# stanford-iprl-lab/nerf_shared

Hardware: AMD Instinct MI355X
Metric: rays_per_sec (higher is better)
Workload: dtype bf16; 1 GPU; lego_halfres_400x400_64c+128f_viewdirs_8x256_chunk4096; entry=Renderer.render(c2w=pose, retraw=False), chunk=4096, N_samples=64, N_importance=128, weights=random-init seeds 0/10, parallelism=single GPU

## Files before the change

include/nerf_amd.h:

```cpp
#ifndef NERF_AMD_H
#define NERF_AMD_H

#include <stdint.h>

#ifdef __cplusplus
extern "C" {
#endif

#define NERF_AMD_ABI_VERSION 7

#define NERF_AMD_OK            0
#define NERF_AMD_EINVAL       -1
#define NERF_AMD_EHIP         -2
#define NERF_AMD_EUNSUPPORTED -3
#define NERF_AMD_ENOMEM       -4

#define NERF_AMD_PREC_FP32 0
#define NERF_AMD_PREC_BF16 1
#define NERF_AMD_PREC_FP32_SPLIT 2

#define NERF_AMD_SPLIT_TRAIN_MAX_POINTS 8388352

#define NERF_AMD_MAX_SKIPS 8

// ... 210 lines not shown
                              void *stream);

int nerf_amd_occupancy_cull(const nerf_amd_occupancy_grid *grid, const float *rays, int32_t ray_ch, const float *z, int64_t R,
                            int32_t S, int32_t *block_counts, int32_t *rank, float *pts_live, float *vd_live, int64_t *count,
                            void *stream);

int nerf_amd_occupancy_expand(const float *raw_live, const int32_t *rank, int64_t n, int32_t ch, float *raw, void *stream);

int nerf_amd_field_points(const nerf_amd_model *m, const float *pts, const float *viewdirs, int64_t n, float *raw,
                          int precision, void *stream);

int64_t nerf_amd_render_rays_culled_workspace(const nerf_amd_render_cfg *cfg, int64_t R, int32_t out_ch);
int     nerf_amd_render_rays_culled(const nerf_amd_render_cfg *cfg, const nerf_amd_model *coarse, const nerf_amd_model *fine,
                                    const nerf_amd_render_io *io, int64_t R, const nerf_amd_occupancy_grid *grid,
                                    int64_t *stats, void *stream);

int nerf_amd_to8b(const float *x, int64_t n, uint8_t *out, void *stream);

int nerf_amd_img2mse(const float *x, const float *y, int64_t n, float *out, float *partials, void *stream);
int nerf_amd_img2mse_backward(const float *x, const float *y, int64_t n, const float *g, float *gx, float *gy, void *stream);

int nerf_amd_assemble_rays(const float *rays_o, const float *rays_d, const float *viewdir_src, int64_t n, float near,
                           float far, float *out, void *stream);

int nerf_amd_adam_step(int32_t n, float *const *params, const float *const *grads, float *const *exp_avg,
                       float *const *exp_avg_sq, const int64_t *numel, int64_t step, double lr, double beta1,
                       double beta2, double eps, double weight_decay, void *stream);

int nerf_amd_adam_step_device(int32_t n, float *const *params, const float *const *grads, float *const *exp_avg,
                              float *const *exp_avg_sq, const int64_t *numel, int64_t *step_dev, const double *lr_dev,
                              double beta1, double beta2, double eps, double weight_decay, float *scalars_dev, void *stream);

int nerf_amd_profile_enable(int on);
int nerf_amd_set_tuning(int key, int value);
int nerf_amd_profile_collect(int64_t launches[3], double total_ms[3], double total_points[3]);

#ifdef __cplusplus
}
#endif
#endif
```

nerf_shared_amd/_lib.py:

```python
import ctypes
import os
from ctypes import POINTER, Structure, c_char_p, c_double, c_float, c_int, c_int32, c_int64, c_uint16, c_uint32, c_void_p

_HERE = os.path.dirname(os.path.abspath(__file__))
LIB_PATH = os.environ.get("NERF_AMD_LIB") or os.path.join(_HERE, "libnerf_amd.so")

ABI_VERSION = 7
PREC_FP32, PREC_BF16, PREC_FP32_SPLIT = 0, 1, 2
COPY_BF16, COPY_BWD, COPY_SPLIT, COPY_BWD_SPLIT, COPY_FP32, COPY_FP32_BWD, COPY_ALL = 1, 2, 4, 8, 16, 32, 63
COPY_BF16_FOLD = 128
COPY_OF = {PREC_BF16: COPY_BF16, PREC_FP32_SPLIT: COPY_SPLIT, PREC_FP32: COPY_FP32}
TRAIN_COPIES = {PREC_BF16: COPY_BF16 | COPY_BWD, PREC_FP32_SPLIT: COPY_SPLIT | COPY_BWD_SPLIT,
                PREC_FP32: COPY_FP32 | COPY_FP32_BWD}
MAX_SKIPS = 8

EXPORTS = (
    "nerf_amd_abi_version", "nerf_amd_last_error",
    "nerf_amd_model_create", "nerf_amd_model_update", "nerf_amd_model_update_copies", "nerf_amd_model_destroy",
    "nerf_amd_model_supports_bf16", "nerf_amd_model_supports_split", "nerf_amd_model_out_ch", "nerf_amd_pack_bf16_host",
    "nerf_amd_embed", "nerf_amd_nerf_forward", "nerf_amd_mlp_embedded", "nerf_amd_ndc_rays", "nerf_amd_raw2outputs", "nerf_amd_raw2outputs_backward", "nerf_amd_sample_pdf",
    "nerf_amd_render_rays_workspace", "nerf_amd_render_rays", "nerf_amd_render_chunks", "nerf_amd_make_rays",
    "nerf_amd_render_batch_workspace", "nerf_amd_render_batch",
    "nerf_amd_profile_enable", "nerf_amd_profile_collect", "nerf_amd_set_tuning",
    "nerf_amd_model_supports_training", "nerf_amd_train_workspace", "nerf_amd_field_forward_train",
    "nerf_amd_field_backward", "nerf_amd_coarse_z", "nerf_amd_resample", "nerf_amd_get_rays_backward", "nerf_amd_to8b", "nerf_amd_ndc_rays_backward", "nerf_amd_adam_step", "nerf_amd_adam_step_device", "nerf_amd_img2mse", "nerf_amd_img2mse_backward", "nerf_amd_assemble_rays",
    "nerf_amd_rays_at_pixels", "nerf_amd_rays_at_pixels_backward", "nerf_amd_se3_transform", "nerf_amd_se3_transform_backward",
    "nerf_amd_field_backward_inputs",
    "nerf_amd_se3_transform_batch", "nerf_amd_se3_transform_batch_backward", "nerf_amd_rays_at_pixels_batch",
    "nerf_amd_rays_at_pixels_batch_backward", "nerf_amd_img2mse_each", "nerf_amd_img2mse_each_backward",
    "nerf_amd_density_arch", "nerf_amd_density", "nerf_amd_density_grad_fused", "nerf_amd_density_grad_workspace",
    "nerf_amd_density_value_grad",
    "nerf_amd_draw_pixels", "nerf_amd_interest_points_workspace", "nerf_amd_interest_points", "nerf_amd_dilate_mask",
    "nerf_amd_compact_mask",
    "nerf_amd_occupancy_query", "nerf_amd_occupancy_sample_points", "nerf_amd_occupancy_mark", "nerf_amd_occupancy_dilate",
    "nerf_amd_occupancy_cull", "nerf_amd_occupancy_expand", "nerf_amd_field_points",
    "nerf_amd_render_rays_culled_workspace", "nerf_amd_render_rays_culled",
)
OCC_OUTSIDE_LIVE, OCC_OUTSIDE_EMPTY = 0, 1


class Arch(Structure):
    _fields_ = [("D", c_int32), ("W", c_int32), ("output_ch", c_int32), ("use_viewdirs", c_int32),
                ("multires", c_int32), ("multires_views", c_int32), ("i_embed", c_int32),
                ("n_skips", c_int32), ("skips", c_int32 * MAX_SKIPS)]


class RenderCfg(Structure):
    _fields_ = [("N_samples", c_int32), ("N_importance", c_int32), ("perturb", c_int32), ("lindisp", c_int32),
                ("white_bkgd", c_int32), ("use_noise", c_int32), ("precision", c_int32), ("reserved", c_int32)]


class RenderIO(Structure):
    _fields_ = [("rays", c_void_p), ("ray_ch", c_int32), ("pad0", c_int32),
                ("t_vals", c_void_p), ("t_rand", c_void_p), ("noise0", c_void_p), ("noise1", c_void_p),
                ("u", c_void_p), ("t_lin_imp", c_void_p), ("z_coarse", c_void_p),
                ("rgb_map", c_void_p), ("disp_map", c_void_p), ("acc_map", c_void_p),
# ... 80 lines not shown
        "nerf_amd_img2mse_each": (c_int, [c_void_p, c_void_p, c_int64, c_int64, c_int32, c_void_p, c_void_p]),
        "nerf_amd_img2mse_each_backward": (c_int, [c_void_p, c_void_p, c_int64, c_int64, c_int32, c_void_p, c_void_p, c_void_p]),
        "nerf_amd_draw_pixels": (c_int, [c_int64, c_int32, c_uint32, c_void_p, c_void_p, c_int32, c_int32, c_void_p, c_int64, c_int32,
                                         c_void_p, c_void_p, c_void_p]),
        "nerf_amd_interest_points_workspace": (c_int64, [c_int32, c_int32]),
        "nerf_amd_interest_points": (c_int, [c_void_p, c_int32, c_int32, c_int32, c_int32, c_void_p, c_void_p, c_void_p]),
        "nerf_amd_dilate_mask": (c_int, [c_void_p, c_int32, c_int32, c_int32, c_int32, c_void_p, c_void_p]),
        "nerf_amd_compact_mask": (c_int, [c_void_p, c_int32, c_int32, c_void_p, c_void_p, c_void_p, c_void_p]),
        "nerf_amd_occupancy_query": (c_int, [POINTER(OccupancyGridC), c_void_p, c_int64, c_void_p, c_void_p, c_void_p]),
        "nerf_amd_occupancy_sample_points": (c_int, [POINTER(OccupancyGridC), c_int64, c_int64, c_int32, c_uint32, c_void_p, c_void_p]),
        "nerf_amd_occupancy_mark": (c_int, [c_void_p, c_int64, c_int64, c_int32, c_float, c_int, c_void_p, c_void_p]),
        "nerf_amd_occupancy_dilate": (c_int, [c_void_p, c_int32, c_int32, c_int32, c_int32, c_void_p, c_void_p]),
        "nerf_amd_occupancy_cull": (c_int, [POINTER(OccupancyGridC), c_void_p, c_int32, c_void_p, c_int64, c_int32, c_void_p, c_void_p,
                                            c_void_p, c_void_p, c_void_p, c_void_p]),
        "nerf_amd_occupancy_expand": (c_int, [c_void_p, c_void_p, c_int64, c_int32, c_void_p, c_void_p]),
        "nerf_amd_field_points": (c_int, [c_void_p, c_void_p, c_void_p, c_int64, c_void_p, c_int, c_void_p]),
        "nerf_amd_render_rays_culled_workspace": (c_int64, [POINTER(RenderCfg), c_int64, c_int32]),
        "nerf_amd_render_rays_culled": (c_int, [POINTER(RenderCfg), c_void_p, c_void_p, POINTER(RenderIO), c_int64,
                                                POINTER(OccupancyGridC), POINTER(c_int64), c_void_p]),
        "nerf_amd_get_rays_backward": (c_int, [c_int32, c_int32, POINTER(c_double), c_int64, c_int64, c_void_p, c_void_p,
                                               c_void_p, c_void_p]),
        "nerf_amd_to8b": (c_int, [c_void_p, c_int64, c_void_p, c_void_p]),
        "nerf_amd_img2mse": (c_int, [c_void_p, c_void_p, c_int64, c_void_p, c_void_p, c_void_p]),
        "nerf_amd_img2mse_backward": (c_int, [c_void_p, c_void_p, c_int64, c_void_p, c_void_p, c_void_p, c_void_p]),
        "nerf_amd_assemble_rays": (c_int, [c_void_p, c_void_p, c_void_p, c_int64, c_float, c_float, c_void_p, c_void_p]),
        "nerf_amd_adam_step": (c_int, [c_int32, c_void_p, c_void_p, c_void_p, c_void_p, c_void_p, c_int64, c_double, c_double,
                               c_double, c_double, c_double, c_void_p]),
        "nerf_amd_adam_step_device": (c_int, [c_int32, c_void_p, c_void_p, c_void_p, c_void_p, c_void_p, c_void_p, c_void_p, c_double,
                                      c_double, c_double, c_double, c_void_p, c_void_p]),
        "nerf_amd_ndc_rays_backward": (c_int, [c_int32, c_int32, c_double, c_float, c_void_p, c_void_p, c_void_p, c_void_p,
                                               c_int64, c_void_p, c_void_p, c_void_p]),
        "nerf_amd_profile_enable": (c_int, [c_int]),
        "nerf_amd_profile_collect": (c_int, [POINTER(c_int64), POINTER(c_double), POINTER(c_double)]),
    }
    for name, (res, args) in sig.items():
        fn = getattr(lib, name)
        fn.restype, fn.argtypes = res, args
    if lib.nerf_amd_abi_version() != ABI_VERSION:
        raise ImportError("libnerf_amd.so ABI version %d, binding expects %d" % (lib.nerf_amd_abi_version(), ABI_VERSION))
    return lib


lib = _load()


class NerfAmdError(RuntimeError):
    pass


def check(rc, what):
    if rc != 0:
        msg = lib.nerf_amd_last_error()
        raise NerfAmdError("%s failed (%d): %s" % (what, rc, msg.decode() if msg else "?"))


def make_arch(D, W, output_ch, skips, use_viewdirs, multires, multires_views, i_embed):
    skips = [int(s) for s in skips]
    if len(skips) > MAX_SKIPS:
        raise ValueError("at most %d skip connections are supported" % MAX_SKIPS)
    a = Arch()
    a.D, a.W, a.output_ch, a.use_viewdirs = int(D), int(W), int(output_ch), int(bool(use_viewdirs))
    a.multires, a.multires_views, a.i_embed, a.n_skips = int(multires), int(multires_views), int(i_embed), len(skips)
    for i, s in enumerate(skips):
        a.skips[i] = s
    return a

# ... 15 lines not shown
```

nerf_shared_amd/csrc/capi.hip:

```cpp
#include <hip/hip_runtime.h>

#include <atomic>
#include <cmath>

#include <cstdio>
#include <cstring>
#include <mutex>
#include <utility>
#include <new>
#include <string>
#include <vector>

#include "kernels.h"
#include "launch_util.h"
#include "program.h"

using namespace na;

namespace {
thread_local std::string g_err;

std::string lds_msg(const char *what, size_t bytes) {
    return std::string(what) + ": the per-ray scratch needs " + std::to_string(bytes) + " bytes of LDS per workgroup, the CU has " +
           std::to_string(LDS_LIMIT_BYTES) + " (fewer samples per ray)";
}

int fail(int code, const std::string &msg) {
    g_err = msg;
    return code;
}
int hip_fail(hipError_t e, const char *what) {
    return fail(NERF_AMD_EHIP, std::string(what) + ": " + hipGetErrorString(e));
}
#define HIP_TRY(expr)                                        \
    do {                                                     \
        hipError_t e_ = (expr);                              \
        if (e_ != hipSuccess) return hip_fail(e_, #expr);    \
    } while (0)

struct ProfRec { hipEvent_t a, b; int cls; double points; };
std::mutex g_prof_mu;
bool g_prof_on = false;
std::vector<ProfRec> g_prof_recs;
std::vector<std::pair<hipEvent_t, hipEvent_t>> g_prof_free;

template <class T>
int upload(T **dst, const std::vector<T> &src) {
    *dst = nullptr;
    if (src.empty()) return NERF_AMD_OK;
    HIP_TRY(hipMalloc(reinterpret_cast<void **>(dst), src.size() * sizeof(T)));
    HIP_TRY(hipMemcpy(*dst, src.data(), src.size() * sizeof(T), hipMemcpyHostToDevice));
    return NERF_AMD_OK;
}
size_t align_up(size_t v) { return (v + 255) & ~(size_t)255; }

constexpr int TILE_CTR_SLOTS = 1024;
unsigned *g_tile_ctr[16] = {};
std::atomic<unsigned> g_tile_ctr_next{0};
}

namespace na {
std::atomic<int> g_variant{0};
std::atomic<int> g_fold{0};

int tile_counters_init(int device) {
    if (device < 0 || device >= 16) return NERF_AMD_EINVAL;
    if (g_tile_ctr[device]) return NERF_AMD_OK;
    unsigned *p = nullptr;
    if (hipMalloc(reinterpret_cast<void **>(&p), TILE_CTR_SLOTS * 2 * sizeof(unsigned)) != hipSuccess) return NERF_AMD_EHIP;
    if (hipMemset(p, 0, TILE_CTR_SLOTS * 2 * sizeof(unsigned)) != hipSuccess) { (void)hipFree(p); return NERF_AMD_EHIP; }
    g_tile_ctr[device] = p;
    return NERF_AMD_OK;
}

unsigned *tile_counter_slot(int device) {
    if (device < 0 || device >= 16 || !g_tile_ctr[device]) return nullptr;
    return g_tile_ctr[device] + 2 * (g_tile_ctr_next.fetch_add(1, std::memory_order_relaxed) % TILE_CTR_SLOTS);
}

unsigned *tile_counter_for(bool deal, hipStream_t s) {
    if (!deal) return nullptr;
    hipStreamCaptureStatus st = hipStreamCaptureStatusNone;
    if (hipStreamIsCapturing(s, &st) != hipSuccess || st != hipStreamCaptureStatusNone) return nullptr;
    int dev = 0;
    return hipGetDevice(&dev) == hipSuccess ? tile_counter_slot(dev) : nullptr;
}
}

struct nerf_amd_model {
    Program prog;
    int device = 0;
    FragDesc *d_frags = nullptr;
    TileDesc *d_tiles = nullptr;
    LayerF32 *d_layers = nullptr;
    TensorDesc *d_tensors = nullptr;
    uint16_t *stream_bf16 = nullptr, *stream_s16 = nullptr, *stream_bwd = nullptr, *stream_split = nullptr;
// ... 1026 lines not shown
    DeviceGuard guard(device);
    if (guard.err != hipSuccess) return hip_fail(guard.err, "hipSetDevice(lane device)");
    SideLane &l = g_lanes[device];
    if (!l.stream) HIP_TRY(hipStreamCreateWithFlags(&l.stream, hipStreamNonBlocking));
    out[0] = l.stream;
    for (int i = 1; i < n; ++i) {
        if (!l.more[i - 1]) HIP_TRY(hipStreamCreateWithFlags(&l.more[i - 1], hipStreamNonBlocking));
        out[i] = l.more[i - 1];
    }
    return NERF_AMD_OK;
}
void lane_release(int device, const std::vector<hipEvent_t> &events) {
    std::lock_guard<std::mutex> lk(g_lane_mu);
    for (hipEvent_t e : events) g_lanes[device].free_events.push_back(e);
}
}
namespace {

nerf_amd_render_io io_rows(const nerf_amd_render_cfg *cfg, const nerf_amd_render_io &io, int64_t r0, int och, void *ws, int64_t ws_bytes) {
    nerf_amd_render_io o = io;
    const int64_t Nc = cfg->N_samples, Ni = cfg->N_importance, Sl = Nc + Ni;
    auto f = [&](const float *p, int64_t row_floats) { return p ? p + r0 * row_floats : nullptr; };
    auto g = [&](float *p, int64_t row_floats) { return p ? p + r0 * row_floats : nullptr; };
    o.rays = f(io.rays, io.ray_ch);
    o.t_rand = f(io.t_rand, Nc); o.noise0 = f(io.noise0, Nc); o.noise1 = f(io.noise1, Sl);
    o.u = f(io.u, Ni); o.z_coarse = f(io.z_coarse, Nc);
    o.rgb_map = g(io.rgb_map, 3); o.disp_map = g(io.disp_map, 1); o.acc_map = g(io.acc_map, 1);
    o.rgb0 = g(io.rgb0, 3); o.disp0 = g(io.disp0, 1); o.acc0 = g(io.acc0, 1); o.z_std = g(io.z_std, 1);
    o.raw = g(io.raw, Sl * och); o.weights = g(io.weights, Sl); o.z_vals = g(io.z_vals, Sl);
    o.workspace = ws; o.workspace_bytes = ws_bytes;
    return o;
}

int64_t n_super_chunks(int64_t N) { return N <= SUPER_CHUNK_RAYS + SUPER_CHUNK_RAYS / 2 ? 1 : (N + SUPER_CHUNK_RAYS - 1) / SUPER_CHUNK_RAYS; }
}

extern "C" {

int64_t nerf_amd_render_batch_workspace(const nerf_amd_render_cfg *cfg, int64_t N, int32_t out_ch) {
    if (!cfg || N < 0) return -1;
    const int64_t n = n_super_chunks(N);
    const int64_t per = nerf_amd_render_rays_workspace(cfg, n == 1 ? N : SUPER_CHUNK_RAYS, out_ch);
    return per * (n < BATCH_SLOTS ? n : BATCH_SLOTS);
}

int nerf_amd_render_batch(const nerf_amd_render_cfg *cfg, const nerf_amd_model *coarse, const nerf_amd_model *fine,
                          const nerf_amd_render_io *io, int64_t N, void *stream) {
    if (!cfg || !coarse || !io || N < 0) return fail(NERF_AMD_EINVAL, "null argument");
    if (N == 0) return NERF_AMD_OK;
    const int64_t n = n_super_chunks(N);
    if (n == 1) return nerf_amd_render_rays(cfg, coarse, fine, io, N, stream);
    const int och = coarse->prog.out_ch;
    const int64_t per = nerf_amd_render_rays_workspace(cfg, SUPER_CHUNK_RAYS, och);
    const int slots = (int)(n < BATCH_SLOTS ? n : BATCH_SLOTS);
    if (!io->workspace || io->workspace_bytes < per * slots) return fail(NERF_AMD_EINVAL, "workspace too small (nerf_amd_render_batch_workspace)");
    if (!io->z_coarse && cfg->perturb && !io->t_rand) return fail(NERF_AMD_EINVAL, "perturb set but neither z_coarse nor t_rand given");

    std::vector<nerf_amd_render_io> ios((size_t)n);
    std::vector<ChunkPlan> plans((size_t)n);
    for (int64_t k = 0; k < n; ++k) {
        const int64_t r0 = k * SUPER_CHUNK_RAYS, R = (k + 1 == n) ? N - r0 : SUPER_CHUNK_RAYS;
        ios[k] = io_rows(cfg, *io, r0, och, static_cast<char *>(io->workspace) + (k % slots) * per, per);
        int rc = plan_chunk(cfg, coarse, fine, &ios[k], R, &plans[k]);
        if (rc) return rc;
    }
    hipStream_t main_s = static_cast<hipStream_t>(stream), side = nullptr;
    const int device = coarse->device;
    const bool two_pass = plans[0].Ni > 0;
    std::vector<hipEvent_t> ev;
    int rc = lane_acquire(device, (int)(3 * n + 1), &side, &ev);
    if (rc) return rc;
    hipEvent_t *ec = ev.data(), *em = ev.data() + n, *ef = ev.data() + 2 * n;
    hipEvent_t start = ev[3 * n];
    auto H = [&](hipError_t e, const char *what) { if (e != hipSuccess && !rc) rc = hip_fail(e, what); };
    H(hipEventRecord(start, main_s), "hipEventRecord");
    H(hipStreamWaitEvent(side, start, 0), "hipStreamWaitEvent");

    auto coarse_field = [&](int64_t k) {
        if (k >= slots) H(hipStreamWaitEvent(main_s, em[k - slots + (two_pass ? 1 : 0)], 0), "hipStreamWaitEvent");
        if (!rc) rc = stage_z(plans[k], main_s);
        if (!rc) rc = stage_field(plans[k], false, main_s);
        H(hipEventRecord(ec[k], main_s), "hipEventRecord");
    };
    if (two_pass) {
        hipStream_t fine_s = main_s;
        hipStream_t lanes2[2];
        if (g_variant == 44 && lane_streams(device, 2, lanes2) == NERF_AMD_OK) {
            fine_s = lanes2[1];
            H(hipStreamWaitEvent(fine_s, start, 0), "hipStreamWaitEvent");
        }
        coarse_field(0);
        for (int64_t k = 0; k < n && !rc; ++k) {
            if (k + 1 < n) coarse_field(k + 1);
            H(hipStreamWaitEvent(side, ec[k], 0), "hipStreamWaitEvent");
            if (k > 0) H(hipStreamWaitEvent(side, ef[k - 1], 0), "hipStreamWaitEvent");
            if (!rc) rc = stage_mid(plans[k], k > 0 ? &plans[k - 1] : nullptr, side);
            H(hipEventRecord(em[k], side), "hipEventRecord");
            H(hipStreamWaitEvent(fine_s, em[k], 0), "hipStreamWaitEvent");
            if (!rc) rc = stage_field(plans[k], true, fine_s);
            H(hipEventRecord(ef[k], fine_s), "hipEventRecord");
        }
        H(hipStreamWaitEvent(side, ef[n - 1], 0), "hipStreamWaitEvent");
        if (!rc) rc = stage_final(plans[n - 1], side);
    } else {
        for (int64_t k = 0; k < n && !rc; ++k) {
            coarse_field(k);
            H(hipStreamWaitEvent(side, ec[k], 0), "hipStreamWaitEvent");
            if (!rc) rc = stage_final(plans[k], side);
            H(hipEventRecord(em[k], side), "hipEventRecord");
        }
    }
    H(hipEventRecord(start, side), "hipEventRecord");
    H(hipStreamWaitEvent(main_s, start, 0), "hipStreamWaitEvent");
    lane_release(device, ev);
    return rc;
}

}

extern "C" {

int nerf_amd_set_tuning(int key, int value) {
    if (key == 0 && value >= 0 && value <= 115) { g_variant.store(value, std::memory_order_relaxed); return NERF_AMD_OK; }
    if (key == 1 && value >= 0 && value <= 1) { g_density_route.store(value, std::memory_order_relaxed); return NERF_AMD_OK; }
    if (key == 2 && value >= 0 && value <= 2) { g_fold.store(value, std::memory_order_relaxed); return NERF_AMD_OK; }
    return fail(NERF_AMD_EINVAL, "unknown tuning key/value");
}

int nerf_amd_profile_enable(int on) {
    std::lock_guard<std::mutex> lk(g_prof_mu);
    g_prof_on = on != 0;
    return NERF_AMD_OK;
}

int nerf_amd_profile_collect(int64_t launches[3], double total_ms[3], double total_points[3]) {
    std::lock_guard<std::mutex> lk(g_prof_mu);
    for (int c = 0; c < 3; ++c) { launches[c] = 0; total_ms[c] = 0.0; total_points[c] = 0.0; }
    for (const ProfRec &r : g_prof_recs) {
        float ms = 0.f;
        if (hipEventSynchronize(r.b) == hipSuccess && hipEventElapsedTime(&ms, r.a, r.b) == hipSuccess) {
            launches[r.cls] += 1; total_ms[r.cls] += ms; total_points[r.cls] += r.points;
        }
        g_prof_free.emplace_back(r.a, r.b);
    }
    g_prof_recs.clear();
    return NERF_AMD_OK;
}

int nerf_amd_get_rays_backward(int32_t H, int32_t W, const double *K4, int64_t pix0, int64_t n, const float *g_rays_o,
                               const float *g_rays_d, float *g_c2w, void *stream) {
    if (H < 1 || W < 1 || !K4 || pix0 < 0 || n < 0 || pix0 + n > (int64_t)H * W || !g_c2w)
        return fail(NERF_AMD_EINVAL, "bad get_rays_backward arguments");
    int rc = launch_get_rays_bwd(H, W, K4, pix0, n, g_rays_o, g_rays_d, g_c2w, static_cast<hipStream_t>(stream));
    return rc ? fail(rc, "get_rays backward launch failed") : NERF_AMD_OK;
}

int nerf_amd_assemble_rays(const float *rays_o, const float *rays_d, const float *viewdir_src, int64_t n, float near,
                           float far, float *out, void *stream) {
    if (n < 0 || (n > 0 && (!rays_o || !rays_d || !out))) return fail(NERF_AMD_EINVAL, "bad assemble_rays arguments");
    int rc = na::launch_assemble_rays(rays_o, rays_d, viewdir_src, n, near, far, out, static_cast<hipStream_t>(stream));
    return rc ? fail(rc, "assemble_rays launch failed") : NERF_AMD_OK;
}

int nerf_amd_adam_step(int32_t n, float *const *params, const float *const *grads, float *const *exp_avg,
                       float *const *exp_avg_sq, const int64_t *numel, int64_t step, double lr, double beta1,
                       double beta2, double eps, double weight_decay, void *stream) {
    if (n < 0 || step < 1 || (n > 0 && (!params || !grads || !exp_avg || !exp_avg_sq || !numel)))
        return fail(NERF_AMD_EINVAL, "bad adam arguments");
    for (int i = 0; i < n; ++i) {
        if (numel[i] < 0 || numel[i] > 0x7fffffff) return fail(NERF_AMD_EINVAL, "adam: tensor size out of range");
        if (numel[i] > 0 && (!params[i] || !grads[i] || !exp_avg[i] || !exp_avg_sq[i])) return fail(NERF_AMD_EINVAL, "adam: null tensor pointer");
    }
    const double bc1 = 1.0 - std::pow(beta1, (double)step), bc2 = 1.0 - std::pow(beta2, (double)step);
    int rc = na::launch_adam(n, params, grads, exp_avg, exp_avg_sq, numel, (float)(lr / bc1), beta1, beta2,
                             (float)eps, (float)weight_decay, (float)std::sqrt(bc2), static_cast<hipStream_t>(stream));
    return rc ? fail(rc, "adam launch failed") : NERF_AMD_OK;
}

int nerf_amd_adam_step_device(int32_t n, float *const *params, const float *const *grads, float *const *exp_avg,
// ... 175 lines not shown
```

nerf_shared_amd/csrc/kernels.h:

```cpp
#pragma once
#include <hip/hip_runtime.h>
#include <stdint.h>
#include <atomic>
#include <vector>

#include "program.h"

namespace na {

struct MlpArgs {
    const uint16_t *stream_bf16;
    const float *bias_bf16;
    const uint16_t *stream_s16;
    const float *bias_s16;
    const uint16_t *stream_split;
    const float *stream_f32;
    const float *bias_f32;
    const LayerF32 *layers;
    int32_t n_layers;
    int32_t input_ch, input_ch_views, W, lds_rows;
    int32_t multires, multires_views, i_embed;
    const float *embedded;
    const float *pts;
    const float *rays;
// ... 86 lines not shown

int launch_adam(int n, float *const *params, const float *const *grads, float *const *exp_avg, float *const *exp_avg_sq,
                const int64_t *numel, float step_size, double beta1, double beta2, float eps, float weight_decay,
                float bc2_sqrt, hipStream_t s, int64_t *step_dev = nullptr, const double *lr_dev = nullptr, float *scalars_dev = nullptr);

struct RenderCfgK {
    int32_t Nc, Ni, perturb, lindisp, white_bkgd;
};
int launch_coarse_z(const float *rays, int ray_stride, const float *t_vals, const float *t_rand,
                    int64_t R, int Nc, int lindisp, int perturb, float *z, hipStream_t s);
int launch_composite(const float *raw, int raw_ch, const float *z, const float *rays_d, int rays_d_stride,
                     const float *noise, int64_t R, int S, int white_bkgd, float *rgb, float *disp, float *acc,
                     float *weights, float *depth, hipStream_t s);
int launch_composite_bwd(const float *raw, int raw_ch, const float *z, const float *rays_d, int rays_d_stride,
                         const float *noise, int64_t R, int S, int white_bkgd, const float *g_rgb, const float *g_disp,
                         const float *g_acc, const float *g_depth, const float *g_weights, float *g_raw, float *g_rays_d,
                         hipStream_t s);
int launch_sample_pdf(const float *bins, const float *weights, const float *u, const float *t_lin,
                      int64_t R, int n_bins, int n_samples, float *samples, hipStream_t s);
int launch_resample(const float *z_coarse, const float *weights, const float *u, const float *t_lin,
                    int64_t R, int Nc, int Ni, float *z_fine, float *z_std, hipStream_t s);
constexpr size_t LDS_LIMIT_BYTES = 160 * 1024;
size_t composite_bwd_lds_bytes(int S);
size_t sample_pdf_lds_bytes(int n_bins);
size_t resample_lds_bytes(int Nc, int Ni, bool with_composite);
struct CompositeJob {
    const float *raw; int raw_ch; const float *z; const float *rays_d; int rays_d_stride; const float *noise;
    int64_t R; int S; int white_bkgd;
    float *rgb, *disp, *acc, *weights;
};
struct ResampleJob {
    const float *u, *t_lin; int Ni, pad_c, pad_s;
    float *z_fine, *z_std;
};
int launch_mid_stage(const CompositeJob &coarse, const ResampleJob &resample, const CompositeJob *final_of_previous_chunk,
                     hipStream_t s);
int launch_ndc_rays_bwd(int H, int W, double focal, float near, const float *rays_o, const float *rays_d, const float *g_oo,
                        const float *g_od, int64_t n, float *g_ro, float *g_rd, hipStream_t s);
int launch_ndc_rays(int H, int W, double focal, float near, const float *rays_o, const float *rays_d, int64_t n,
                    float *out_o, float *out_d, hipStream_t s);
int launch_get_rays_bwd(int H, int W, const double *K4, int64_t pix0, int64_t n, const float *g_o, const float *g_d,
                        float *g_c2w, hipStream_t s);
int launch_to8b(const float *x, int64_t n, uint8_t *out, hipStream_t s);
int launch_make_rays(int H, int W, const double *K4, const float *c2w, const float *c2w_static,
                     int64_t pix0, int64_t n, float near, float far, int use_viewdirs, int ndc,
                     float *rays_out, hipStream_t s);
constexpr int RAYS_AT_BWD_PER_BLOCK = 16384, RAYS_AT_BWD_MAX_BLOCKS = 256;
constexpr int POSE_BATCH_MAX = 1024, IMG2MSE_EACH_MAX = 16384;
int launch_se3_transform(const float *w, const float *v, const float *theta, const float *x, int x_stride, int B, float *T,
                         hipStream_t s);
int launch_se3_transform_bwd(const float *w, const float *v, const float *theta, const float *x, int x_stride, int B, const float *g_T,
                             float *g_w, float *g_v, float *g_theta, hipStream_t s);
int launch_rays_at_pixels(const double *K4, const float *c2w, int64_t c2w_pose_stride, int c2w_row_stride, int B, const int32_t *pix,
                          int64_t n, float *rays_o, float *rays_d, hipStream_t s);
int launch_rays_at_pixels_bwd(const double *K4, const int32_t *pix, int64_t n, int B, const float *g_o, const float *g_d, float *g_c2w,
                              float *partials, hipStream_t s);
int launch_img2mse(const float *x, const float *y, int64_t y_stride, int64_t n, int B, float *out, float *partials, hipStream_t s);
int launch_img2mse_bwd(const float *x, const float *y, int64_t y_stride, int64_t n, int B, const float *g, float *gx, float *gy,
                       hipStream_t s);
int launch_draw_pixels(int64_t M, int n, uint32_t seed, int64_t *draw_count, const int32_t *region, int W, const float *image,
                       int64_t row_stride, int C, int32_t *pixels, float *target, hipStream_t s);
int launch_interest_points(const uint8_t *image, int H, int W, int C, int quality, void *workspace, uint8_t *mask, hipStream_t s);
int launch_dilate_mask(const uint8_t *in, int H, int W, int k, int iterations, uint8_t *out, hipStream_t s);
int launch_compact_mask(const uint8_t *mask, int H, int W, int32_t *block_counts, int32_t *list, int64_t *count, hipStream_t s);
int launch_compact_scan(int32_t *block_counts, int n_blocks, int64_t *count, hipStream_t s);

// ... 17 lines not shown
```

nerf_shared_amd/csrc/launch_util.h:

```cpp
#pragma once
#include <hip/hip_runtime.h>

#include <atomic>
#include <cstdint>

#include "kernels.h"

namespace na {

extern std::atomic<int> g_variant;

constexpr int MAX_TRACKED_DEVICES = 64;

inline int current_device() {
    int d = 0;
    return hipGetDevice(&d) == hipSuccess ? d : -1;
}

inline int device_cu_count() {
    static std::atomic<int> cache[MAX_TRACKED_DEVICES];
    const int dev = current_device();
    const bool tracked = dev >= 0 && dev < MAX_TRACKED_DEVICES;
    if (tracked) {
        const int c = cache[dev].load(std::memory_order_relaxed);
        if (c > 0) return c;
    }
    int n = 0;
    if (dev < 0 || hipDeviceGetAttribute(&n, hipDeviceAttributeMultiprocessorCount, dev) != hipSuccess || n <= 0) n = 256;
    if (tracked) cache[dev].store(n, std::memory_order_relaxed);
    return n;
}

struct DynamicLdsOptIn {
    std::atomic<uint64_t> done{0};
    hipError_t ensure(const void *kernel, size_t bytes) {
        const int dev = current_device();
        const bool tracked = dev >= 0 && dev < MAX_TRACKED_DEVICES;
        const uint64_t bit = tracked ? (uint64_t)1 << dev : 0;
        if (tracked && (done.load(std::memory_order_acquire) & bit)) return hipSuccess;
        const hipError_t e = hipFuncSetAttribute(kernel, hipFuncAttributeMaxDynamicSharedMemorySize, (int)bytes);
        if (e == hipSuccess && tracked) done.fetch_or(bit, std::memory_order_release);
        return e;
    }
// ... 59 lines not shown
```

nerf_shared_amd/csrc/render.hip:

```cpp
#include <hip/hip_runtime.h>
#include <cstring>
#include <math.h>

#include "kernels.h"
#include "launch_util.h"

namespace na {

constexpr int RAYS_PER_WG = 4;

constexpr size_t LDS_PER_CU = 160 * 1024;
static int pow2_at_least(int n) {
    int p = 2;
    while (p < n) p <<= 1;
    return p;
}
size_t composite_bwd_lds_bytes(int S) { return (size_t)RAYS_PER_WG * 3 * S * sizeof(float); }
size_t sample_pdf_lds_bytes(int n_bins) { return (size_t)RAYS_PER_WG * 2 * n_bins * sizeof(float); }
size_t resample_lds_bytes(int Nc, int Ni, bool with_composite) {
    return (size_t)RAYS_PER_WG * ((with_composite ? Nc : 0) + 2 * (size_t)(Nc - 1) + pow2_at_least(Nc) + pow2_at_least(Ni)) * sizeof(float);
}
static int reserve_lds(DynamicLdsOptIn &opt_in, const void *kernel, size_t bytes) {
    if (bytes > LDS_PER_CU) return NERF_AMD_EINVAL;
    if (bytes > 64 * 1024 && opt_in.ensure(kernel, LDS_PER_CU) != hipSuccess) return NERF_AMD_EHIP;
// ... 330 lines not shown
    const size_t lds = sample_pdf_lds_bytes(n_bins);
    static DynamicLdsOptIn opt_in;
    if (int rc = reserve_lds(opt_in, reinterpret_cast<const void *>(sample_pdf_kernel), lds)) return rc;
    hipLaunchKernelGGL(sample_pdf_kernel, dim3((unsigned)blocks), dim3(64 * RAYS_PER_WG), lds, s, bins, weights, u,
                       t_lin, R, n_bins, n_samples, samples);
    return hipGetLastError() == hipSuccess ? NERF_AMD_OK : NERF_AMD_EHIP;
}

__device__ __forceinline__ unsigned order_key(float v) {
    const unsigned b = __builtin_bit_cast(unsigned, v);
    return (b & 0x80000000u) ? ~b : (b | 0x80000000u);
}

__device__ __forceinline__ bool wave_is_sorted(const float *x, int n, int lane) {
    bool ok = true;
    for (int i = lane; i + 1 < n; i += 64) ok = ok && order_key(x[i]) <= order_key(x[i + 1]);
    return __all(ok);
}

__device__ __forceinline__ void wave_bitonic_sort(float *x, int npad, int lane) {
    for (int k = 2; k <= npad; k <<= 1) {
        for (int j = k >> 1; j > 0; j >>= 1) {
            for (int t = lane; t < (npad >> 1); t += 64) {
                const int i = ((t & ~(j - 1)) << 1) | (t & (j - 1));
                const float a = x[i], b = x[i + j];
                const bool up = (i & k) == 0;
                if ((order_key(a) > order_key(b)) == up) { x[i] = b; x[i + j] = a; }
            }
            wave_lds_sync();
        }
    }
}

template <bool STRICT>
__device__ __forceinline__ int count_below(const float *x, int n, unsigned k) {
    int lo = 0, hi = n;
    while (lo < hi) {
        const int mid = (lo + hi) >> 1;
        const unsigned km = order_key(x[mid]);
        if (STRICT ? km < k : km <= k) lo = mid + 1; else hi = mid;
    }
    return lo;
}

template <class LoadW>
__device__ __forceinline__ void resample_ray(const float *z_coarse, LoadW load_w, const float *u, const float *t_lin,
                                             int64_t r, bool live, int Nc, int Ni, int pad_c, int pad_s, float *scratch,
                                             float *z_fine, float *z_std, int lane) {
    const int nb = Nc - 1;
    float *cdf = scratch, *bl = cdf + nb, *za = bl + nb, *zs = za + pad_c;
    const float *zr = z_coarse + r * Nc;
    build_cdf(load_w, nb, cdf, lane);
    for (int i = lane; i < nb; i += 64) bl[i] = 0.5f * (zr[i + 1] + zr[i]);
    for (int i = lane; i < pad_c; i += 64) za[i] = i < Nc ? zr[i] : INFINITY;
    for (int i = Ni + lane; i < pad_s; i += 64) zs[i] = INFINITY;
    wave_lds_sync();
    double sum = 0.0;
    for (int i = lane; i < Ni; i += 64) {
        const float uu = u ? u[r * Ni + i] : t_lin[i];
        const float v = invert_cdf(cdf, bl, nb, uu);
        zs[i] = v;
        sum += (double)v;
    }
    const double mean = wave_sum(sum) / (double)Ni;
    double ss = 0.0;
    for (int i = lane; i < Ni; i += 64) {
        const double dv = (double)zs[i] - mean;
        ss += dv * dv;
    }
    ss = wave_sum(ss);
    if (live && lane == 0 && z_std) z_std[r] = (float)sqrt(ss / (double)Ni);
    wave_lds_sync();
    if (!wave_is_sorted(zs, Ni, lane)) wave_bitonic_sort(zs, pad_s, lane);
    if (!wave_is_sorted(za, Nc, lane)) wave_bitonic_sort(za, pad_c, lane);
    if (!live) return;
    float *out = z_fine + r * (Nc + Ni);
    for (int i = lane; i < Nc; i += 64) {
        const float v = za[i];
        out[i + count_below<true>(zs, Ni, order_key(v))] = v;
    }
    for (int j = lane; j < Ni; j += 64) {
        const float v = zs[j];
        out[j + count_below<false>(za, Nc, order_key(v))] = v;
    }
}

__global__ __launch_bounds__(64 * RAYS_PER_WG) void resample_kernel(const float *z_coarse, const float *weights,
                                                                    const float *u, const float *t_lin, int64_t R,
                                                                    int Nc, int Ni, int pad_c, int pad_s, float *z_fine,
                                                                    float *z_std) {
    extern __shared__ float lds[];
    const int lane = threadIdx.x & 63, wv = threadIdx.x >> 6;
    int64_t r = (int64_t)blockIdx.x * RAYS_PER_WG + wv;
    const bool live = r < R;
    if (!live) r = R - 1;
    const float *wr = weights + r * Nc + 1;
    resample_ray(z_coarse, [&](int i) { return wr[i]; }, u, t_lin, r, live, Nc, Ni, pad_c, pad_s,
                 lds + wv * (2 * (Nc - 1) + pad_c + pad_s), z_fine, z_std, lane);
}

__global__ __launch_bounds__(64 * RAYS_PER_WG) void mid_stage_kernel(CompositeJob cj, ResampleJob rj, CompositeJob fj,
                                                                     int cr_blocks) {
    extern __shared__ float lds[];
    const int lane = threadIdx.x & 63, wv = threadIdx.x >> 6;
    if ((int)blockIdx.x < cr_blocks) {
        int64_t r = (int64_t)blockIdx.x * RAYS_PER_WG + wv;
        const bool live = r < cj.R;
        if (!live) r = cj.R - 1;
        const int Nc = cj.S;
        float *wl = lds + wv * (Nc + 2 * (Nc - 1) + rj.pad_c + rj.pad_s);
        composite_ray(cj.raw, cj.raw_ch, cj.z, cj.rays_d, cj.rays_d_stride, cj.noise, r, Nc, cj.white_bkgd,
                      live ? cj.rgb : nullptr, live ? cj.disp : nullptr, live ? cj.acc : nullptr, nullptr, lane,
                      [&](int s, float w) { wl[s] = w; if (live && cj.weights) cj.weights[r * Nc + s] = w; });
        wave_lds_sync();
        resample_ray(cj.z, [&](int i) { return wl[1 + i]; }, rj.u, rj.t_lin, r, live, Nc, rj.Ni, rj.pad_c, rj.pad_s,
                     wl + Nc, rj.z_fine, rj.z_std, lane);
    } else {
        const int64_t r = (int64_t)((int)blockIdx.x - cr_blocks) * RAYS_PER_WG + wv;
        if (r >= fj.R) return;
        composite_ray(fj.raw, fj.raw_ch, fj.z, fj.rays_d, fj.rays_d_stride, fj.noise, r, fj.S, fj.white_bkgd, fj.rgb, fj.disp,
                      fj.acc, nullptr, lane, [&](int s, float w) { if (fj.weights) fj.weights[r * fj.S + s] = w; });
    }
}

int launch_mid_stage(const CompositeJob &cj, const ResampleJob &rj, const CompositeJob *fj, hipStream_t s) {
    if (cj.R <= 0) return NERF_AMD_EINVAL;
    const int Nc = cj.S, Ni = rj.Ni;
    if (cj.raw_ch < 4 || Nc < 3 || Ni < 1) return NERF_AMD_EINVAL;
    ResampleJob r2 = rj;
    r2.pad_c = pow2_at_least(Nc); r2.pad_s = pow2_at_least(Ni);
    CompositeJob f2;
    std::memset(&f2, 0, sizeof(f2));
    if (fj) f2 = *fj;
    const int64_t cr_blocks = (cj.R + RAYS_PER_WG - 1) / RAYS_PER_WG;
    const int64_t f_blocks = (f2.R + RAYS_PER_WG - 1) / RAYS_PER_WG;
    if (cr_blocks + f_blocks >= ((int64_t)1 << 31)) return NERF_AMD_EINVAL;
    const size_t lds = resample_lds_bytes(Nc, Ni, true);
    static DynamicLdsOptIn opt_in;
    if (int rc = reserve_lds(opt_in, reinterpret_cast<const void *>(mid_stage_kernel), lds)) return rc;
    hipLaunchKernelGGL(mid_stage_kernel, dim3((unsigned)(cr_blocks + f_blocks)), dim3(64 * RAYS_PER_WG), lds, s, cj, r2, f2,
                       (int)cr_blocks);
    return hipGetLastError() == hipSuccess ? NERF_AMD_OK : NERF_AMD_EHIP;
}

int launch_resample(const float *z_coarse, const float *weights, const float *u, const float *t_lin,
                    int64_t R, int Nc, int Ni, float *z_fine, float *z_std, hipStream_t s) {
    if (R <= 0) return NERF_AMD_OK;
    if (Nc < 3 || Ni < 1) return NERF_AMD_EINVAL;
    const int pad_c = pow2_at_least(Nc), pad_s = pow2_at_least(Ni);
    const int64_t blocks = (R + RAYS_PER_WG - 1) / RAYS_PER_WG;
    const size_t lds = resample_lds_bytes(Nc, Ni, false);
    static DynamicLdsOptIn opt_in;
    if (int rc = reserve_lds(opt_in, reinterpret_cast<const void *>(resample_kernel), lds)) return rc;
    hipLaunchKernelGGL(resample_kernel, dim3((unsigned)blocks), dim3(64 * RAYS_PER_WG), lds, s, z_coarse, weights, u,
                       t_lin, R, Nc, Ni, pad_c, pad_s, z_fine, z_std);
    return hipGetLastError() == hipSuccess ? NERF_AMD_OK : NERF_AMD_EHIP;
}

__device__ __forceinline__ float norm3(float x, float y, float z) { return sqrtf((x * x + z * z) + y * y); }

struct RayGen {
    float fx, fy, cx, cy;
    float c2w[12], c2ws[12];
    int has_static, use_viewdirs, ndc, H, W;
    float near, far;
    float sx, sy;
};

__device__ __forceinline__ void cam_ray(const float *c, float dx, float dy, float dz, float *o, float *d) {
#pragma unroll
    for (int k = 0; k < 3; ++k) {
        d[k] = dx * c[4 * k] + dy * c[4 * k + 1] + dz * c[4 * k + 2];
        o[k] = c[4 * k + 3];
    }
}

__global__ __launch_bounds__(256) void make_rays_kernel(RayGen g, int64_t pix0, int64_t n, float *out) {
    const int64_t idx = (int64_t)blockIdx.x * blockDim.x + threadIdx.x;
    if (idx >= n) return;
    const int64_t pix = pix0 + idx;
    const float i = (float)(pix % g.W), j = (float)(pix / g.W);
    const float dx = (i - g.cx) / g.fx, dy = -(j - g.cy) / g.fy, dz = -1.0f;
    float o[3], d[3], vd[3];
    cam_ray(g.c2w, dx, dy, dz, o, d);
    vd[0] = d[0]; vd[1] = d[1]; vd[2] = d[2];
    if (g.has_static) cam_ray(g.c2ws, dx, dy, dz, o, d);
    const int ch = g.use_viewdirs ? 11 : 8;
    float *row = out + idx * ch;
// ... 482 lines not shown
```

Baseline: 5.662 million rays/s.

## Reorder batch pipeline so mid stage issues before next coarse field; add tunable lag and register sort

The two-pass batch loop now enqueues the mid stage (coarse composite plus resample) for chunk k before launching chunk k+1's coarse field, and makes the lag between a chunk's fine field and its final composite tunable, defaulting to the previous value of 1. Tail finalisation loops over the last `lag` chunks. The change also adds an optional register-resident bitonic sort for the fine samples, off by default, and a profiling API that reports the union of kernel time spans. The reordering is meant to let the side stream start resampling sooner and overlap better with the main-stream field evaluation. The rotation now depends on BATCH_SLOTS exceeding the lag.

```diff
diff --git a/include/nerf_amd.h b/include/nerf_amd.h
--- a/include/nerf_amd.h
+++ b/include/nerf_amd.h
@@ -266,6 +266,7 @@
                               double beta1, double beta2, double eps, double weight_decay, float *scalars_dev, void *stream);
 
 int nerf_amd_profile_enable(int on);
+int nerf_amd_profile_collect_spans(int64_t launches[3], double union_ms[3], double sum_ms[3], double total_points[3]);
 int nerf_amd_set_tuning(int key, int value);
 int nerf_amd_profile_collect(int64_t launches[3], double total_ms[3], double total_points[3]);
 
diff --git a/nerf_shared_amd/_lib.py b/nerf_shared_amd/_lib.py
--- a/nerf_shared_amd/_lib.py
+++ b/nerf_shared_amd/_lib.py
@@ -21,7 +21,7 @@
     "nerf_amd_embed", "nerf_amd_nerf_forward", "nerf_amd_mlp_embedded", "nerf_amd_ndc_rays", "nerf_amd_raw2outputs", "nerf_amd_raw2outputs_backward", "nerf_amd_sample_pdf",
     "nerf_amd_render_rays_workspace", "nerf_amd_render_rays", "nerf_amd_render_chunks", "nerf_amd_make_rays",
     "nerf_amd_render_batch_workspace", "nerf_amd_render_batch",
-    "nerf_amd_profile_enable", "nerf_amd_profile_collect", "nerf_amd_set_tuning",
+    "nerf_amd_profile_enable", "nerf_amd_profile_collect", "nerf_amd_profile_collect_spans", "nerf_amd_set_tuning",
     "nerf_amd_model_supports_training", "nerf_amd_train_workspace", "nerf_amd_field_forward_train",
     "nerf_amd_field_backward", "nerf_amd_coarse_z", "nerf_amd_resample", "nerf_amd_get_rays_backward", "nerf_amd_to8b", "nerf_amd_ndc_rays_backward", "nerf_amd_adam_step", "nerf_amd_adam_step_device", "nerf_amd_img2mse", "nerf_amd_img2mse_backward", "nerf_amd_assemble_rays",
     "nerf_amd_rays_at_pixels", "nerf_amd_rays_at_pixels_backward", "nerf_amd_se3_transform", "nerf_amd_se3_transform_backward",
@@ -168,6 +168,7 @@
                                                c_int64, c_void_p, c_void_p, c_void_p]),
         "nerf_amd_profile_enable": (c_int, [c_int]),
         "nerf_amd_profile_collect": (c_int, [POINTER(c_int64), POINTER(c_double), POINTER(c_double)]),
+        "nerf_amd_profile_collect_spans": (c_int, [POINTER(c_int64), POINTER(c_double), POINTER(c_double), POINTER(c_double)]),
     }
     for name, (res, args) in sig.items():
         fn = getattr(lib, name)
diff --git a/nerf_shared_amd/csrc/capi.hip b/nerf_shared_amd/csrc/capi.hip
--- a/nerf_shared_amd/csrc/capi.hip
+++ b/nerf_shared_amd/csrc/capi.hip
@@ -11,6 +11,7 @@
 #include <string>
 #include <vector>
 
+#include "interval_union.h"
 #include "kernels.h"
 #include "launch_util.h"
 #include "program.h"
@@ -43,6 +44,7 @@
 bool g_prof_on = false;
 std::vector<ProfRec> g_prof_recs;
 std::vector<std::pair<hipEvent_t, hipEvent_t>> g_prof_free;
+hipEvent_t g_prof_ref = nullptr;
 
 template <class T>
 int upload(T **dst, const std::vector<T> &src) {
@@ -62,6 +64,8 @@
 namespace na {
 std::atomic<int> g_variant{0};
 std::atomic<int> g_fold{0};
+std::atomic<int> g_final_lag{0};
+std::atomic<int> g_fine_sort{0};
 
 int tile_counters_init(int device) {
     if (device < 0 || device >= 16) return NERF_AMD_EINVAL;
@@ -1154,6 +1158,20 @@
     return o;
 }
 
+constexpr int DEFAULT_FINAL_LAG = 1;
+constexpr bool DEFAULT_FINE_STREAM = false;
+int batch_final_lag() {
+    static_assert(BATCH_SLOTS > 2, "a group's workspace is in use for `lag` groups after its own: the rotation needs more slots than that");
+    const int v = g_final_lag.load(std::memory_order_relaxed);
+    return v ? v : DEFAULT_FINAL_LAG;
+}
+bool batch_fine_stream(hipStream_t main_s) {
+    const int v = g_variant.load(std::memory_order_relaxed);
+    if (!(v == 44 || (v != 45 && DEFAULT_FINE_STREAM))) return false;
+    hipStreamCaptureStatus st = hipStreamCaptureStatusNone;
+    return hipStreamIsCapturing(main_s, &st) == hipSuccess && st == hipStreamCaptureStatusNone;
+}
+
 int64_t n_super_chunks(int64_t N) { return N <= SUPER_CHUNK_RAYS + SUPER_CHUNK_RAYS / 2 ? 1 : (N + SUPER_CHUNK_RAYS - 1) / SUPER_CHUNK_RAYS; }
 }
 
@@ -1198,8 +1216,9 @@
     H(hipEventRecord(start, main_s), "hipEventRecord");
     H(hipStreamWaitEvent(side, start, 0), "hipStreamWaitEvent");
 
+    const int lag = !two_pass ? 0 : batch_final_lag();
     auto coarse_field = [&](int64_t k) {
-        if (k >= slots) H(hipStreamWaitEvent(main_s, em[k - slots + (two_pass ? 1 : 0)], 0), "hipStreamWaitEvent");
+        if (k >= slots) H(hipStreamWaitEvent(main_s, em[k - slots + lag], 0), "hipStreamWaitEvent");
         if (!rc) rc = stage_z(plans[k], main_s);
         if (!rc) rc = stage_field(plans[k], false, main_s);
         H(hipEventRecord(ec[k], main_s), "hipEventRecord");
@@ -1207,23 +1226,25 @@
     if (two_pass) {
         hipStream_t fine_s = main_s;
         hipStream_t lanes2[2];
-        if (g_variant == 44 && lane_streams(device, 2, lanes2) == NERF_AMD_OK) {
+        if (batch_fine_stream(main_s) && lane_streams(device, 2, lanes2) == NERF_AMD_OK) {
             fine_s = lanes2[1];
             H(hipStreamWaitEvent(fine_s, start, 0), "hipStreamWaitEvent");
         }
         coarse_field(0);
         for (int64_t k = 0; k < n && !rc; ++k) {
+            H(hipStreamWaitEvent(side, ec[k], 0), "hipStreamWaitEvent");
+            if (k >= lag) H(hipStreamWaitEvent(side, ef[k - lag], 0), "hipStreamWaitEvent");
+            if (!rc) rc = stage_mid(plans[k], k >= lag ? &plans[k - lag] : nullptr, side);
+            H(hipEventRecord(em[k], side), "hipEventRecord");
             if (k + 1 < n) coarse_field(k + 1);
-            H(hipStreamWaitEvent(side, ec[k], 0), "hipStreamWaitEvent");
-            if (k > 0) H(hipStreamWaitEvent(side, ef[k - 1], 0), "hipStreamWaitEvent");
-            if (!rc) rc = stage_mid(plans[k], k > 0 ? &plans[k - 1] : nullptr, side);
-            H(hipEventRecord(em[k], side), "hipEventRecord");
             H(hipStreamWaitEvent(fine_s, em[k], 0), "hipStreamWaitEvent");
             if (!rc) rc = stage_field(plans[k], true, fine_s);
             H(hipEventRecord(ef[k], fine_s), "hipEventRecord");
         }
-        H(hipStreamWaitEvent(side, ef[n - 1], 0), "hipStreamWaitEvent");
-        if (!rc) rc = stage_final(plans[n - 1], side);
+        for (int64_t j = n > lag ? n - lag : 0; j < n && !rc; ++j) {
+            H(hipStreamWaitEvent(side, ef[j], 0), "hipStreamWaitEvent");
+            rc = stage_final(plans[j], side);
+        }
     } else {
         for (int64_t k = 0; k < n && !rc; ++k) {
             coarse_field(k);
@@ -1246,27 +1267,45 @@
     if (key == 0 && value >= 0 && value <= 115) { g_variant.store(value, std::memory_order_relaxed); return NERF_AMD_OK; }
     if (key == 1 && value >= 0 && value <= 1) { g_density_route.store(value, std::memory_order_relaxed); return NERF_AMD_OK; }
     if (key == 2 && value >= 0 && value <= 2) { g_fold.store(value, std::memory_order_relaxed); return NERF_AMD_OK; }
+    if (key == 3 && value >= 0 && value <= 2) { g_final_lag.store(value, std::memory_order_relaxed); return NERF_AMD_OK; }
+    if (key == 4 && value >= 0 && value <= 2) { g_fine_sort.store(value, std::memory_order_relaxed); return NERF_AMD_OK; }
     return fail(NERF_AMD_EINVAL, "unknown tuning key/value");
 }
 
 int nerf_amd_profile_enable(int on) {
     std::lock_guard<std::mutex> lk(g_prof_mu);
+    if (on && !g_prof_on) {
+        if (!g_prof_ref) HIP_TRY(hipEventCreate(&g_prof_ref));
+        HIP_TRY(hipEventRecord(g_prof_ref, nullptr));
+    }
     g_prof_on = on != 0;
     return NERF_AMD_OK;
 }
 
-int nerf_amd_profile_collect(int64_t launches[3], double total_ms[3], double total_points[3]) {
+int nerf_amd_profile_collect_spans(int64_t launches[3], double union_ms[3], double sum_ms[3], double total_points[3]) {
     std::lock_guard<std::mutex> lk(g_prof_mu);
-    for (int c = 0; c < 3; ++c) { launches[c] = 0; total_ms[c] = 0.0; total_points[c] = 0.0; }
+    std::vector<std::pair<double, double>> spans[3];
+    double unplaced_ms[3] = {0.0, 0.0, 0.0};
+    for (int c = 0; c < 3; ++c) { launches[c] = 0; union_ms[c] = 0.0; sum_ms[c] = 0.0; total_points[c] = 0.0; }
+    const bool have_ref = g_prof_ref && hipEventSynchronize(g_prof_ref) == hipSuccess;
     for (const ProfRec &r : g_prof_recs) {
-        float ms = 0.f;
+        float ms = 0.f, at = 0.f;
         if (hipEventSynchronize(r.b) == hipSuccess && hipEventElapsedTime(&ms, r.a, r.b) == hipSuccess) {
-            launches[r.cls] += 1; total_ms[r.cls] += ms; total_points[r.cls] += r.points;
+            launches[r.cls] += 1; sum_ms[r.cls] += ms; total_points[r.cls] += r.points;
+            if (have_ref && hipEventElapsedTime(&at, g_prof_ref, r.a) == hipSuccess) spans[r.cls].emplace_back((double)at, (double)at + (double)ms);
+            else unplaced_ms[r.cls] += ms;
         }
         g_prof_free.emplace_back(r.a, r.b);
     }
     g_prof_recs.clear();
+    (void)hipGetLastError();
+    for (int c = 0; c < 3; ++c) union_ms[c] = na::interval_union_measure(spans[c]) + unplaced_ms[c];
     return NERF_AMD_OK;
+}
+
+int nerf_amd_profile_collect(int64_t launches[3], double total_ms[3], double total_points[3]) {
+    double sum_ms[3];
+    return nerf_amd_profile_collect_spans(launches, total_ms, sum_ms, total_points);
 }
 
 int nerf_amd_get_rays_backward(int32_t H, int32_t W, const double *K4, int64_t pix0, int64_t n, const float *g_rays_o,
diff --git a/nerf_shared_amd/csrc/interval_union.h b/nerf_shared_amd/csrc/interval_union.h
--- /dev/null
+++ b/nerf_shared_amd/csrc/interval_union.h
@@ -0,0 +1,19 @@
+#pragma once
+#include <algorithm>
+#include <utility>
+#include <vector>
+
+namespace na {
+inline double interval_union_measure(std::vector<std::pair<double, double>> &iv) {
+    std::sort(iv.begin(), iv.end());
+    double total = 0.0, lo = 0.0, hi = 0.0;
+    bool open = false;
+    for (const auto &[a, b] : iv) {
+        if (!(b > a)) continue;
+        if (open && a <= hi) { hi = std::max(hi, b); continue; }
+        if (open) total += hi - lo;
+        lo = a; hi = b; open = true;
+    }
+    return open ? total + (hi - lo) : total;
+}
+}
diff --git a/nerf_shared_amd/csrc/kernels.h b/nerf_shared_amd/csrc/kernels.h
--- a/nerf_shared_amd/csrc/kernels.h
+++ b/nerf_shared_amd/csrc/kernels.h
@@ -142,6 +142,7 @@
 struct ResampleJob {
     const float *u, *t_lin; int Ni, pad_c, pad_s;
     float *z_fine, *z_std;
+    int sort_regs;
 };
 int launch_mid_stage(const CompositeJob &coarse, const ResampleJob &resample, const CompositeJob *final_of_previous_chunk,
                      hipStream_t s);
diff --git a/nerf_shared_amd/csrc/launch_util.h b/nerf_shared_amd/csrc/launch_util.h
--- a/nerf_shared_amd/csrc/launch_util.h
+++ b/nerf_shared_amd/csrc/launch_util.h
@@ -9,6 +9,7 @@
 namespace na {
 
 extern std::atomic<int> g_variant;
+extern std::atomic<int> g_fine_sort;
 
 constexpr int MAX_TRACKED_DEVICES = 64;
 
diff --git a/nerf_shared_amd/csrc/render.hip b/nerf_shared_amd/csrc/render.hip
--- a/nerf_shared_amd/csrc/render.hip
+++ b/nerf_shared_amd/csrc/render.hip
@@ -386,6 +386,42 @@
     }
 }
 
+constexpr int REG_SORT_MAX = 256;
+template <int E>
+__device__ __forceinline__ void wave_bitonic_sort_regs(float *x, int npad, int lane) {
+    float v[E];
+#pragma unroll
+    for (int e = 0; e < E; ++e) v[e] = lane + 64 * e < npad ? x[lane + 64 * e] : __builtin_bit_cast(float, 0x7fffffffu);
+#pragma unroll
+    for (int k = 2; k <= 64 * E; k <<= 1) {
+#pragma unroll
+        for (int j = k >> 1; j > 0; j >>= 1) {
+            if (j >= 64) {
+#pragma unroll
+                for (int e = 0; e < E; ++e) {
+                    if (e & (j >> 6)) continue;
+                    const float a = v[e], b = v[e + (j >> 6)];
+                    const bool up = ((64 * e) & k) == 0;
+                    const bool swap = (order_key(a) > order_key(b)) == up;
+                    v[e] = swap ? b : a; v[e + (j >> 6)] = swap ? a : b;
+                }
+            } else {
+#pragma unroll
+                for (int e = 0; e < E; ++e) {
+                    const float a = v[e], b = __shfl_xor(a, j);
+                    const bool keep_min = ((lane & j) == 0) == (((lane + 64 * e) & k) == 0);
+                    const unsigned ka = order_key(a), kb = order_key(b);
+                    v[e] = (keep_min ? kb < ka : kb > ka) ? b : a;
+                }
+            }
+        }
+    }
+#pragma unroll
+    for (int e = 0; e < E; ++e)
+        if (lane + 64 * e < npad) x[lane + 64 * e] = v[e];
+    wave_lds_sync();
+}
+
 template <bool STRICT>
 __device__ __forceinline__ int count_below(const float *x, int n, unsigned k) {
     int lo = 0, hi = n;
@@ -399,8 +435,8 @@
 
 template <class LoadW>
 __device__ __forceinline__ void resample_ray(const float *z_coarse, LoadW load_w, const float *u, const float *t_lin,
-                                             int64_t r, bool live, int Nc, int Ni, int pad_c, int pad_s, float *scratch,
-                                             float *z_fine, float *z_std, int lane) {
+                                             int64_t r, bool live, int Nc, int Ni, int pad_c, int pad_s, bool sort_regs,
+                                             float *scratch, float *z_fine, float *z_std, int lane) {
     const int nb = Nc - 1;
     float *cdf = scratch, *bl = cdf + nb, *za = bl + nb, *zs = za + pad_c;
     const float *zr = z_coarse + r * Nc;
@@ -425,7 +461,12 @@
     ss = wave_sum(ss);
     if (live && lane == 0 && z_std) z_std[r] = (float)sqrt(ss / (double)Ni);
     wave_lds_sync();
-    if (!wave_is_sorted(zs, Ni, lane)) wave_bitonic_sort(zs, pad_s, lane);
+    if (!wave_is_sorted(zs, Ni, lane)) {
+        if (!sort_regs) wave_bitonic_sort(zs, pad_s, lane);
+        else if (pad_s <= 64) wave_bitonic_sort_regs<1>(zs, pad_s, lane);
+        else if (pad_s <= 128) wave_bitonic_sort_regs<2>(zs, pad_s, lane);
+        else wave_bitonic_sort_regs<4>(zs, pad_s, lane);
+    }
     if (!wave_is_sorted(za, Nc, lane)) wave_bitonic_sort(za, pad_c, lane);
     if (!live) return;
     float *out = z_fine + r * (Nc + Ni);
@@ -441,15 +482,15 @@
 
 __global__ __launch_bounds__(64 * RAYS_PER_WG) void resample_kernel(const float *z_coarse, const float *weights,
                                                                     const float *u, const float *t_lin, int64_t R,
-                                                                    int Nc, int Ni, int pad_c, int pad_s, float *z_fine,
-                                                                    float *z_std) {
+                                                                    int Nc, int Ni, int pad_c, int pad_s, int sort_regs,
+                                                                    float *z_fine, float *z_std) {
     extern __shared__ float lds[];
     const int lane = threadIdx.x & 63, wv = threadIdx.x >> 6;
     int64_t r = (int64_t)blockIdx.x * RAYS_PER_WG + wv;
     const bool live = r < R;
     if (!live) r = R - 1;
     const float *wr = weights + r * Nc + 1;
-    resample_ray(z_coarse, [&](int i) { return wr[i]; }, u, t_lin, r, live, Nc, Ni, pad_c, pad_s,
+    resample_ray(z_coarse, [&](int i) { return wr[i]; }, u, t_lin, r, live, Nc, Ni, pad_c, pad_s, sort_regs != 0,
                  lds + wv * (2 * (Nc - 1) + pad_c + pad_s), z_fine, z_std, lane);
 }
 
@@ -468,13 +509,19 @@
                       [&](int s, float w) { wl[s] = w; if (live && cj.weights) cj.weights[r * Nc + s] = w; });
         wave_lds_sync();
         resample_ray(cj.z, [&](int i) { return wl[1 + i]; }, rj.u, rj.t_lin, r, live, Nc, rj.Ni, rj.pad_c, rj.pad_s,
-                     wl + Nc, rj.z_fine, rj.z_std, lane);
+                     rj.sort_regs != 0, wl + Nc, rj.z_fine, rj.z_std, lane);
     } else {
         const int64_t r = (int64_t)((int)blockIdx.x - cr_blocks) * RAYS_PER_WG + wv;
         if (r >= fj.R) return;
         composite_ray(fj.raw, fj.raw_ch, fj.z, fj.rays_d, fj.rays_d_stride, fj.noise, r, fj.S, fj.white_bkgd, fj.rgb, fj.disp,
                       fj.acc, nullptr, lane, [&](int s, float w) { if (fj.weights) fj.weights[r * fj.S + s] = w; });
     }
+}
+
+constexpr bool DEFAULT_SORT_REGS = false;
+static int sort_in_registers(int pad_s) {
+    const int v = g_fine_sort.load(std::memory_order_relaxed);
+    return pad_s <= REG_SORT_MAX && (v ? v == 2 : DEFAULT_SORT_REGS);
 }
 
 int launch_mid_stage(const CompositeJob &cj, const ResampleJob &rj, const CompositeJob *fj, hipStream_t s) {
@@ -483,6 +530,7 @@
     if (cj.raw_ch < 4 || Nc < 3 || Ni < 1) return NERF_AMD_EINVAL;
     ResampleJob r2 = rj;
     r2.pad_c = pow2_at_least(Nc); r2.pad_s = pow2_at_least(Ni);
+    r2.sort_regs = sort_in_registers(r2.pad_s);
     CompositeJob f2;
     std::memset(&f2, 0, sizeof(f2));
     if (fj) f2 = *fj;
@@ -507,7 +555,7 @@
     static DynamicLdsOptIn opt_in;
     if (int rc = reserve_lds(opt_in, reinterpret_cast<const void *>(resample_kernel), lds)) return rc;
     hipLaunchKernelGGL(resample_kernel, dim3((unsigned)blocks), dim3(64 * RAYS_PER_WG), lds, s, z_coarse, weights, u,
-                       t_lin, R, Nc, Ni, pad_c, pad_s, z_fine, z_std);
+                       t_lin, R, Nc, Ni, pad_c, pad_s, sort_in_registers(pad_s), z_fine, z_std);
     return hipGetLastError() == hipSuccess ? NERF_AMD_OK : NERF_AMD_EHIP;
 }
 
```

New measurement: 5.660 million rays/s. No clear change (-0.0%).
